# LittleWat/multichannel-semseg-with-uda

Hardware: AMD Instinct MI355X
Metric: RGB-D img/s (6x480x640) MCD train step, drn_d_38 (higher is better)
Workload: dtype f32 (operands split 2-way into scaled fp16, 3 cross terms on the fp16 MFMA pipe, fp32 accumulate)

## Files before the change

multichannel-semseg-with-uda_amd/csrc/conv_gemm_split_pp.hip:

```cpp
#include <cstdlib>
#include <type_traits>

#include "conv_split_params.h"
#include "options.h"

namespace {

template <class P, bool DGRAD, int WM, int WN, int QM, int QN>
__global__ __launch_bounds__(512, (WM * WN <= 4 ? 4 : 2)) void conv_gemm_split_pp_kernel(ConvSplitParams p) {
  static_assert(QM * QN == 4, "four waves per group");
  constexpr int WAVES_N = QN;
  constexpr int BM = 2 * QM * WM * 32, BN = QN * WN * 32, NT = 512, NS = 3;
  constexpr int NP = P::NP;
  constexpr int NPU = P::NPU;
  constexpr int NQ = 2 * NP;
  typedef typename P::frag frag;
  constexpr int A_UNITS = 2 * NPU * BM;
  constexpr int A_DMAS = (A_UNITS + NT - 1) / NT;
  constexpr int B_UNITS = 2 * NPU * BN;
  constexpr int B_DMAS = (B_UNITS + NT - 1) / NT;
  constexpr int KDEEP = P::KDEEP;
  static_assert(KDEEP == 1 || NPU == 1, "deep K-steps use the slots of the pieces the policy does not stage");
  constexpr int A_SUB = 2 * NPU * BM > A_DMAS * NT ? 2 * NPU * BM : A_DMAS * NT;
  constexpr int B_SUB = 2 * NPU * BN > B_DMAS * NT ? 2 * NPU * BN : B_DMAS * NT;
  constexpr int DMA_PER_STEP = KDEEP * (A_DMAS + B_DMAS);
  constexpr int A_BYTES = KDEEP > 1 ? KDEEP * A_SUB * 16 : (NQ * BM > A_DMAS * NT ? NQ * BM : A_DMAS * NT) * 16;
  constexpr int B_BYTES = KDEEP > 1 ? KDEEP * B_SUB * 16 : (NQ * BN > B_DMAS * NT ? NQ * BN : B_DMAS * NT) * 16;
  constexpr bool SAMEPX = (NT % BN) == 0;
  constexpr int NPX = SAMEPX ? 1 : B_DMAS;
  constexpr bool LANEHALF = (BN % 64) != 0;
  static_assert(BM % 64 == 0 && (2 * BN) % 64 == 0 && (!LANEHALF || !SAMEPX),
                "every wave issues the same number of DMAs (the waits are counted); a wave's units share a piece");
  static_assert(NS * (A_BYTES + B_BYTES) <= 160 * 1024, "LDS");

  __shared__ __attribute__((aligned(16))) unsigned char smem[NS * (A_BYTES + B_BYTES)];
  unsigned char* As = smem;
  unsigned char* Bs = smem + NS * A_BYTES;

  const int t = threadIdx.x;
  const int lane = t & 63;
  const int wave = __builtin_amdgcn_readfirstlane(t >> 6);
  const int grp_id = wave >> 2;
  const int wm = grp_id * QM + (wave & 3) / QN;
  const int wn = (wave & 3) % QN;
  const int l31 = lane & 31, lh = lane >> 5;

  const int m_tiles = p.Mp / BM;
  const int n_tiles = p.tile_n1;
  const int per_xcd = (n_tiles - p.tile_n0 + 7) >> 3;
  const int xcd = blockIdx.x & 7;
  const int slot = blockIdx.x >> 3;
  const int tile_m = slot % m_tiles;
  const int tile_n = p.tile_n0 + xcd * per_xcd + slot / m_tiles;
  if (tile_n >= n_tiles) return;

  const int HWd = p.Hd * p.Wd;
  const int HWs = p.Hs * p.Ws;
  constexpr unsigned OOB = 0x80000000u;
  __amdgpu_buffer_rsrc_t cb_rs[NPU];
#pragma unroll
  for (int pc = 0; pc < NPU; ++pc)
    cb_rs[pc] = __builtin_amdgcn_make_buffer_rsrc((void*)((const char*)p.src_cb + pc * p.cb_piece_stride), 0, p.cb_bytes, 0x00020000);
  const __amdgpu_buffer_rsrc_t wp_rs = __builtin_amdgcn_make_buffer_rsrc((void*)p.wp, 0, p.wp_bytes, 0x00020000);
  const int C8 = p.Cs >> 3;
  const int taps = p.KH * p.KW;
  unsigned valid_mask[NPX], vbase[NPX];
  int khalf[NPX];
#pragma unroll
  for (int x = 0; x < NPX; ++x) {
    const int plane_l = (t + x * NT) / BN;
    khalf[x] = LANEHALF ? (plane_l & 1) : 0;
    const int bj = (t + x * NT) % BN;
    const int pix = tile_n * BN + bj;
    const bool pv = pix < p.P;
    int pn = 0, py = 0, px = 0;
    if (pv) {
      pn = pix / HWd;
      const int rem = pix - pn * HWd;
      py = rem / p.Wd;
      px = rem - py * p.Wd;
    }
    const unsigned pix_base = (unsigned)pn * (unsigned)C8 * (unsigned)HWs;
    unsigned vm = 0;
    for (int q = 0; q < taps; ++q) {
      const int ky = q / p.KW, kx = q - ky * p.KW;
      const int sy = DGRAD ? py + p.pad - ky * p.dil : py * p.stride + ky * p.dil - p.pad;
      const int sx = DGRAD ? px + p.pad - kx * p.dil : px * p.stride + kx * p.dil - p.pad;
      vm |= (pv && sy >= 0 && sy < p.Hs && sx >= 0 && sx < p.Ws ? 1u : 0u) << q;
    }
    valid_mask[x] = (LANEHALF && plane_l >= 2 * NPU) ? 0u : vm;
    vbase[x] = DGRAD ? pix_base + (unsigned)(py * p.Ws + px) : pix_base + (unsigned)(py * p.stride * p.Ws + px * p.stride);
    if (LANEHALF) vbase[x] += (unsigned)(khalf[x] * HWs);
  }

  unsigned a_voff[A_DMAS];
#pragma unroll
  for (int i = 0; i < A_DMAS; ++i) {
    const int id = t + i * NT;
    const int plane = id / BM;
    const int m = id - plane * BM;
    a_voff[i] = id < A_UNITS ? ((unsigned)plane * (unsigned)p.Mp + (unsigned)m) * 16u : OOB;
  }

  int l_tap = 0, l_c0 = 0, l_ky = 0, l_kx = 0, l_kstep = 0;
  auto issue_sub = [&](int buf, int d) {
#if defined(__HIP_DEVICE_COMPILE__)
    const int a_soff = (l_kstep * NQ * p.Mp + tile_m * BM) * 16;
    unsigned char* adst = As + buf * A_BYTES + (d * A_SUB + wave * 64) * 16;
#pragma unroll
    for (int i = 0; i < A_DMAS; ++i)
      __builtin_amdgcn_raw_ptr_buffer_load_lds(wp_rs, (__attribute__((address_space(3))) void*)(adst + i * NT * 16), 16, a_voff[i], a_soff, 0, 0);
    const int rel = DGRAD ? (p.pad - l_ky * p.dil) * p.Ws + (p.pad - l_kx * p.dil) : (l_ky * p.dil - p.pad) * p.Ws + (l_kx * p.dil - p.pad);
    unsigned voff[NPX];
#pragma unroll
    for (int x = 0; x < NPX; ++x) {
      bool ok = ((valid_mask[x] >> l_tap) & 1u) != 0;
      if (LANEHALF) ok = ok && (l_c0 >> 3) + khalf[x] < C8;
      voff[x] = ok ? (vbase[x] + (unsigned)rel) * 16u : OOB;
    }
#if defined(MCD_ABLATE) && (MCD_ABLATE & 64)
    if (l_tap == 0)
#endif
#pragma unroll
    for (int i = 0; i < B_DMAS; ++i) {
      const int unit0 = wave * 64 + i * NT;
      const int plane = LANEHALF ? 2 * (unit0 / (2 * BN)) : unit0 / BN;
      const int grp = (l_c0 >> 3) + (plane & 1);
      const int soff = (grp < C8 && plane < 2 * NPU) ? grp * HWs * 16 : 0x7FFFFFFF;
      unsigned char* bdst = Bs + buf * B_BYTES + (d * B_SUB + unit0) * 16;
      const __amdgpu_buffer_rsrc_t rs = (NPU > 1 && plane >= 2) ? cb_rs[NPU - 1] : cb_rs[0];
      __builtin_amdgcn_raw_ptr_buffer_load_lds(rs, (__attribute__((address_space(3))) void*)bdst, 16, voff[SAMEPX ? 0 : i], soff, 0, 0);
    }
#else
    (void)buf;
    (void)d;
#endif
  };
  auto advance = [&]() {
    ++l_kstep;
    ++l_tap;
    if (++l_kx == p.KW) {
      l_kx = 0;
      ++l_ky;
    }
    if (l_tap == taps) {
      l_tap = 0;
      l_kx = 0;
      l_ky = 0;
      l_c0 += 16;
    }
  };

  auto issue = [&](int buf) {
    issue_sub(buf, 0);
    if constexpr (KDEEP > 1) {
#pragma unroll
      for (int d = 1; d < KDEEP; ++d) {
        advance();
        issue_sub(buf, d);
      }
    }
  };

  f32x16 acc[WM][WN];
#pragma unroll
  for (int i = 0; i < WM; ++i)
#pragma unroll
    for (int j = 0; j < WN; ++j)
#pragma unroll
      for (int r = 0; r < 16; ++r) acc[i][j][r] = 0.f;

  const int nsteps = taps * (p.Kp / 16) / KDEEP;
  issue(0);
  if (nsteps > 1) {
    advance();
    issue(1);
  }
  asm volatile("s_waitcnt vmcnt(0) lgkmcnt(0)\n\ts_barrier" ::: "memory");
  if (grp_id == 1) __builtin_amdgcn_s_barrier();

  frag fa[KDEEP > 1 ? KDEEP : NP][WM], fb[KDEEP > 1 ? KDEEP : NP][WN];
  int cur = 0, nxt2 = 2;
  for (int s = 0; s < nsteps; ++s) {
    const unsigned char* a_base = As + cur * A_BYTES + (lh * BM + wm * (32 * WM) + l31) * 16;
    const unsigned char* b_base = Bs + cur * B_BYTES + (lh * BN + wn * (32 * WN) + l31) * 16;
    if constexpr (KDEEP > 1) {
#pragma unroll
      for (int d = 0; d < KDEEP; ++d) {
#pragma unroll
        for (int i = 0; i < WM; ++i) fa[d][i] = *reinterpret_cast<const frag*>(a_base + (d * A_SUB + i * 32) * 16);
#pragma unroll
        for (int j = 0; j < WN; ++j) fb[d][j] = *reinterpret_cast<const frag*>(b_base + (d * B_SUB + j * 32) * 16);
      }
    } else {
#pragma unroll
    for (int pc = 0; pc < NPU; ++pc) {
#pragma unroll
      for (int i = 0; i < WM; ++i) fa[pc][i] = *reinterpret_cast<const frag*>(a_base + (pc * 2 * BM + i * 32) * 16);
#pragma unroll
      for (int j = 0; j < WN; ++j) fb[pc][j] = *reinterpret_cast<const frag*>(b_base + (pc * 2 * BN + j * 32) * 16);
    }
    }
    __builtin_amdgcn_sched_barrier(0);
    if (s + 2 < nsteps) {
      advance();
      issue(nxt2);
      asm volatile("s_waitcnt vmcnt(%0) lgkmcnt(0)\n\ts_barrier" ::"n"(DMA_PER_STEP) : "memory");
    } else {
      asm volatile("s_waitcnt vmcnt(0) lgkmcnt(0)\n\ts_barrier" ::: "memory");
    }
    __builtin_amdgcn_sched_barrier(0);
    if constexpr (KDEEP > 1) {
#pragma unroll
      for (int d = 0; d < KDEEP; ++d)
#pragma unroll
        for (int i = 0; i < WM; ++i)
#pragma unroll
          for (int j = 0; j < WN; ++j) acc[i][j] = P::mfma(fa[d][i], fb[d][j], acc[i][j]);
    } else {
#pragma unroll
    for (int tm = 0; tm < P::NTERMS; ++tm)
#pragma unroll
      for (int i = 0; i < WM; ++i)
#pragma unroll
        for (int j = 0; j < WN; ++j) acc[i][j] = P::mfma(fa[P::TA[tm]][i], fb[P::TB[tm]][j], acc[i][j]);
    }
    __builtin_amdgcn_sched_barrier(0);
    asm volatile("s_barrier" ::: "memory");
    cur = cur == 2 ? 0 : cur + 1;
    nxt2 = nxt2 == 2 ? 0 : nxt2 + 1;
  }
  if (grp_id == 0) __builtin_amdgcn_s_barrier();

  if constexpr (P::SCALED) {
    const float osc = mcd_scale_of_bound(*p.src_bound) * mcd_scale_of_bound(*p.w_bound);
#pragma unroll
    for (int i = 0; i < WM; ++i)
#pragma unroll
      for (int j = 0; j < WN; ++j)
#pragma unroll
        for (int r = 0; r < 16; ++r) acc[i][j][r] *= osc;
  }
  const int m_wave = tile_m * BM + wm * (32 * WM);
  const int p_wave = tile_n * BN + wn * (32 * WN);
  if (!DGRAD && p.bias != nullptr) {
#pragma unroll
    for (int i = 0; i < WM; ++i)
#pragma unroll
      for (int r = 0; r < 16; ++r) {
        const int m = m_wave + i * 32 + (r & 3) + 8 * (r >> 2) + 4 * lh;
        const float bv = (m < p.M) ? p.bias[m] : 0.f;
#pragma unroll
        for (int j = 0; j < WN; ++j) acc[i][j][r] += bv;
      }
  }
// ... 223 lines not shown
  return math == MCDSEG_MATH_F16X1 && !small && mcd_opt(MCD_OPT_PP_DEEP) != 0 && ((q.KH * q.KW * (q.Kp / 16)) & 1) == 0;
}

template <int WM, int WN, int QM, int QN>
void launch_math(const ConvSplitParams& q, int math, bool dgrad, hipStream_t st) {
  if constexpr (!(WM == 2 && WN == 2 && QM == 2 && QN == 2)) {
    if (deep_applies<WM, WN, QM, QN>(q, math)) {
      if (dgrad)
        launch_tile<SplitF16x1D, true, WM, WN, QM, QN>(q, st);
      else
        launch_tile<SplitF16x1D, false, WM, WN, QM, QN>(q, st);
      return;
    }
  }
  if (math == MCDSEG_MATH_F16X1) {
    if (dgrad)
      launch_tile<SplitF16x1, true, WM, WN, QM, QN>(q, st);
    else
      launch_tile<SplitF16x1, false, WM, WN, QM, QN>(q, st);
  } else {
    if (dgrad)
      launch_tile<SplitF16x3, true, WM, WN, QM, QN>(q, st);
    else
      launch_tile<SplitF16x3, false, WM, WN, QM, QN>(q, st);
  }
}

int pp_wide(const ConvSplitParams& p, int math, bool dgrad) {
  const int mode = pp_mode();
  if ((mode != 3 && mode != 4) || !pp_applies(p, math, dgrad, 128)) return 0;
  const int kind = (p.Mp % 256) == 0 ? 1 : 2;
  if (mode == 4) return kind;
  const int64_t fill = mcd_opt(MCD_OPT_PP_WIDE_FILL);
  if (fill > 100) return 0;
  const int64_t cus = compute_units();
  if (kind == 2) {
    if (mcd_opt(MCD_OPT_PP_WIDE128) == 0) return 0;
    const int64_t tiles = ceil_div64(p.P, 320) * (p.Mp / 128), rounds_w = ceil_div64(tiles, cus);
    return tiles * 100 >= fill * rounds_w * cus ? 2 : 0;
  }
  const int64_t m_tiles = p.Mp / 256;
  const int64_t tiles = ceil_div64(p.P, 320) * m_tiles, rounds_w = ceil_div64(tiles, cus);
  const int min_rounds = pp_min_rounds() > 1 ? pp_min_rounds() : 1;
  const int64_t rounds = (p.P / 256) * m_tiles / cus;
  if (rounds < min_rounds) {
    if (tiles * 100 >= fill * rounds_w * cus) return 1;
    const int64_t tiles_h = ceil_div64(p.P, 160) * m_tiles, rounds_h = ceil_div64(tiles_h, cus);
    return tiles_h * 100 >= fill * rounds_h * cus ? 3 : 0;
  }
  int64_t n_pp = rounds * cus / m_tiles;
  if (n_pp > p.P / 256) n_pp = p.P / 256;
  const int64_t rest = ceil_div64(p.P - n_pp * 256, 128) * m_tiles;
  return 5 * rounds_w <= 4 * rounds + 2 * ceil_div64(rest, cus) ? 1 : 0;
}

}

int mcdseg_internal_conv_pp_wide(const ConvSplitParams& p, int math, bool dgrad) { return pp_wide(p, math, dgrad); }

int mcdseg_internal_conv_pp_deep(const ConvSplitParams& p, int math) { return deep_applies<4, 2, 1, 4>(p, math) ? 1 : 0; }

int64_t mcdseg_internal_conv_pp_pixels(const ConvSplitParams& p, int math, bool dgrad) {
  const int mode = pp_mode();
  if (pp_wide(p, math, dgrad)) return p.P;
  if ((mode != 1 && mode != 3) || !pp_applies(p, math, dgrad)) return 0;
  const int64_t m_tiles = p.Mp / 256, n_full = p.P / 256, cus = compute_units();
  const int64_t rounds = n_full * m_tiles / cus;
  if (rounds < 1 || rounds < pp_min_rounds()) return 0;
  int64_t n_pp = rounds * cus / m_tiles;
  if (n_pp > n_full) n_pp = n_full;
  return n_pp * 256;
}

int mcdseg_internal_conv_pp_rest(const ConvSplitParams& p, int math, bool dgrad) {
  const int mode = pp_mode();
  if (!pp_applies(p, math, dgrad)) return 0;
  if (mode == 2) return 1;
  return mode == 3 && (p.P / 256) * (p.Mp / 256) / compute_units() >= (pp_min_rounds() > 1 ? pp_min_rounds() : 1) ? 1 : 0;
}

int mcdseg_internal_conv_pp_launch(const ConvSplitParams& p, int math, bool dgrad, int64_t pixels, hipStream_t st) {
  ConvSplitParams q = p;
  q.sub = 0;
  q.tile_n0 = 0;
  if (const int kind = pp_wide(p, math, dgrad)) {
    q.tile_n1 = ceil_div(p.P, kind == 3 ? 160 : 320);
    if (kind == 1)
      launch_math<2, 5, 2, 2>(q, math, dgrad, st);
    else if (kind == 2)
      launch_math<1, 5, 2, 2>(q, math, dgrad, st);
    else
      launch_math<1, 5, 4, 1>(q, math, dgrad, st);
    MCD_LAUNCH_CHECK("conv_gemm_split_pp (256 / 128 x 320, 256 x 160)");
    return 0;
  }
  q.tile_n1 = (int)(pixels / 256);
  launch_math<4, 2, 1, 4>(q, math, dgrad, st);
  MCD_LAUNCH_CHECK("conv_gemm_split_pp");
  return 0;
}

int mcdseg_internal_conv_pp_rest_launch(const ConvSplitParams& p, int math, bool dgrad, int64_t pix0, hipStream_t st) {
  ConvSplitParams q = p;
  q.sub = 0;
  q.tile_n0 = (int)(pix0 / 128);
  q.tile_n1 = ceil_div(p.P, 128);
  launch_math<2, 2, 2, 2>(q, math, dgrad, st);
  MCD_LAUNCH_CHECK("conv_gemm_split_pp (256 x 128)");
  return 0;
}
```

multichannel-semseg-with-uda_amd/csrc/conv_split_params.h:

```cpp
#pragma once
#include "split.h"

struct ConvSplitParams {
  const float* src;
  const void* src_cb;
  const void* wp;
  const float* src_bound;
  const float* w_bound;
  const float* bias;
  float* dst;
  float* stats;
  const float* ep_scale;
  const float* ep_shift;
  const float* ep_res;
  int ep_relu;
  int N;
  int Cs, Hs, Ws;
  int M, Hd, Wd;
  int Mp, Kp;
  int KH, KW, stride, pad, dil;
  int P;
  int src_bytes, wp_bytes, cb_bytes;
  long long cb_piece_stride;
  int sub;
  int cls_tile0[5];
  int tile_n0, tile_n1;
  int ep_res_lds;
  unsigned ep_res_bytes;
  void* dst16;
  float* dst_bound;
  const void* ep_res16;
};

typedef _Float16 mcd_f16x4 __attribute__((ext_vector_type(4)));
typedef __bf16 mcd_bf16x4 __attribute__((ext_vector_type(4)));
```

multichannel-semseg-with-uda_amd/csrc/conv_wgrad_split_pp.hip:

```cpp
#include <cstdlib>
#include <type_traits>

#include "split.h"

namespace {

struct WgradPpParams {
  const void* x_cb;
  const void* dy_cb;
  float* slab;
  int N, Cin, H, W, Cout, Ho, Wo;
  int KH, KW, stride, pad, dil;
  int co_tiles, ci_tiles;
  int tiles_x, tiles_y;
  int kt;
  int L, nwg;
  int slabs;
  int items;
  int x_cb_bytes, dy_cb_bytes;
  long long x_piece_stride, dy_piece_stride;
};

template <class P>
__global__ __launch_bounds__(512) void conv_wgrad_split_pp_kernel(WgradPpParams p) {
  static_assert(P::NP == 2, "two-piece policies");
  constexpr int WM = 4, WN = 2;
  constexpr int NP = P::NP;
  constexpr int NBLK = 2;
  typedef typename P::frag frag;
  typedef short s16x4 __attribute__((ext_vector_type(4)));
  typedef short s16x8 __attribute__((ext_vector_type(8)));
  constexpr int NDMA = 4;
  constexpr int DSTR = 1024 + 64;
  constexpr int BLKB = NDMA * DSTR;
  constexpr int UNIT = NBLK * BLKB;
  constexpr int STAGE = 2 * NP * UNIT;
  constexpr int NS = 3;
  static_assert(NS * STAGE <= 160 * 1024, "LDS");
  constexpr bool DEEP = P::KDEEP == 2 && P::NPU == 1 && NP == 2;
  constexpr int PRO = DEEP ? 4 : 2;
  __shared__ __attribute__((aligned(16))) unsigned char smem[NS * STAGE];

  const int t = threadIdx.x;
  const int lane = t & 63;
  const int wave = __builtin_amdgcn_readfirstlane(t >> 6);
  const int grp_id = wave >> 2;
  const int wm = grp_id, wn = wave & 3;
  const int l31 = lane & 31, lh = lane >> 5;
  const int T_ = p.KH * p.KW;

  const int w_id = (blockIdx.x & 7) * (gridDim.x >> 3) + (blockIdx.x >> 3);
  if (w_id >= p.nwg) return;
  const int tiles_all = p.co_tiles * p.ci_tiles * T_;
  const long long total = (long long)tiles_all * p.kt;
  long long g_next = (long long)w_id * p.L;
  long long g_end = g_next + p.L;
  if (g_end > total) g_end = total;
  int item = w_id;
  if (p.slabs > 0) {
    g_next = 0;
    g_end = item < p.items ? 1 : 0;
  }

  const int opnd = wave >> 2;
  const int piece = (wave >> 1) & 1;
  const int blk = wave & 1;
  const bool isx = opnd == 1;
  const int px = lane & 15;
  const int cgl = lane >> 4;
  const int sH = isx ? p.H : p.Ho;
  const int sW = isx ? p.W : p.Wo;
  const int sS = isx ? p.stride : 1;
  const int sC8 = (isx ? p.Cin : p.Cout) >> 3;
  const int sHW = sH * sW;
  const int bias = p.pad * 16 + 16;
  const char* sptr = (const char*)(isx ? p.x_cb : p.dy_cb) + piece * (isx ? p.x_piece_stride : p.dy_piece_stride) - bias;
  const int sbytes = (isx ? p.x_cb_bytes : p.dy_cb_bytes) + bias;
  const __amdgpu_buffer_rsrc_t rs = __builtin_amdgcn_make_buffer_rsrc((void*)sptr, 0, sbytes, 0x00020000);
  constexpr unsigned OOB = 0x80000000u;
  const int lane_x = px * sS;
  unsigned char* const unit_lds = smem + (opnd * NP + piece) * UNIT + blk * BLKB;
  const bool dma_on = piece < P::NPU;
  const int ntiles = p.tiles_x * p.tiles_y;

  const int gl = lane & 15;
  const int tq = gl >> 2, tpp = gl & 3;
  const int trow = ((((lane >> 4) & 1) * 2 + (tpp >> 1)) * DSTR) + tq * 16 + 8 * (tpp & 1) + (2 * lh) * 64;
  const int a_lane = wm * BLKB + trow;
  const int b_lane = (wn >> 1) * BLKB + (wn & 1) * 512 + trow;

  auto tr_read_at = [&](unsigned base, auto off_c) -> s16x4 {
    s16x4 v;
#if defined(__HIP_DEVICE_COMPILE__)
    asm volatile("ds_read_b64_tr_b16 %0, %1 offset:%2" : "=v"(v) : "v"(base), "n"(decltype(off_c)::value) : "memory");
#else
    (void)base;
    v = s16x4{};
#endif
    return v;
  };
  auto frag_of = [&](unsigned base, auto lo_c, auto hi_c) -> frag {
    const s16x4 lo = tr_read_at(base, lo_c);
    const s16x4 hi = tr_read_at(base, hi_c);
    const s16x8 v = {lo[0], lo[1], lo[2], lo[3], hi[0], hi[1], hi[2], hi[3]};
    return __builtin_bit_cast(frag, v);
  };
#if defined(__HIP_DEVICE_COMPILE__)
  const unsigned smem_lds = (unsigned)(size_t)(__attribute__((address_space(3))) unsigned char*)smem;
#else
  const unsigned smem_lds = 0;
#endif

  while (g_next < g_end) {
    int tile, k0, k1, slab_id;
    if (p.slabs > 0) {
      const int sl = item / tiles_all;
      tile = item - sl * tiles_all;
      k0 = sl * p.L;
      k1 = k0 + p.L < p.kt ? k0 + p.L : p.kt;
      slab_id = item;
      item += p.nwg;
      if (item >= p.items) g_next = g_end;
    } else {
      tile = (int)(g_next / p.kt);
      k0 = (int)(g_next - (long long)tile * p.kt);
      k1 = (g_end - (long long)tile * p.kt < p.kt) ? (int)(g_end - (long long)tile * p.kt) : p.kt;
      slab_id = (int)(g_next / p.L) + tile;
      g_next += k1 - k0;
    }
    const int tap = tile % T_;
    const int tile_ci = (tile / T_) % p.ci_tiles;
    const int tile_co = tile / (T_ * p.ci_tiles);
    const int ky = tap / p.KW, kx = tap - ky * p.KW;
    const int shy = isx ? ky * p.dil - p.pad : 0;
    const int shx = isx ? kx * p.dil - p.pad : 0;
    const int cg0 = (isx ? tile_ci : tile_co) * 32 + blk * 16;
    unsigned vconst[NDMA];
#pragma unroll
    for (int d = 0; d < NDMA; ++d) vconst[d] = (cg0 + d + 4 * cgl) < sC8 ? (unsigned)((d + 4 * cgl) * sHW + px * sS) * 16u : OOB;

    int l_n = k0 / ntiles;
    int l_ty = (k0 - l_n * ntiles) / p.tiles_x;
    int l_tx = k0 - l_n * ntiles - l_ty * p.tiles_x;
    auto stage_off = [](int c) { return DEEP ? (c < NS ? c * STAGE : (c - NS) * STAGE + UNIT) : c * STAGE; };
    auto issue = [&](int stage) {
#if defined(__HIP_DEVICE_COMPILE__)
      if (dma_on) {
        const int sbase = (l_n * sC8 + cg0) * sHW;
        const int iy = l_ty * sS + shy;
        const int ux = l_tx * 16 * sS + shx;
        const bool colok = (unsigned)(ux + lane_x) < (unsigned)sW;
        const int soff = ((unsigned)iy < (unsigned)sH) ? (sbase + iy * sW + ux) * 16 + bias : 0x7FFFFFFF;
#pragma unroll
        for (int d = 0; d < NDMA; ++d)
          __builtin_amdgcn_raw_ptr_buffer_load_lds(rs, (__attribute__((address_space(3))) void*)(unit_lds + stage_off(stage) + d * DSTR), 16,
                                                   colok ? vconst[d] : OOB, soff, 0, 0);
      }
#else
      (void)stage;
#endif
    };
    auto advance = [&]() {
      if (++l_tx == p.tiles_x) {
        l_tx = 0;
        if (++l_ty == p.tiles_y) {
          l_ty = 0;
          ++l_n;
        }
      }
    };

    f32x16 acc[WM][WN];
#pragma unroll
    for (int i = 0; i < WM; ++i)
#pragma unroll
      for (int j = 0; j < WN; ++j)
#pragma unroll
        for (int r = 0; r < 16; ++r) acc[i][j][r] = 0.f;

    const int nsteps = k1 - k0;
    issue(0);
#pragma unroll
    for (int a = 1; a < PRO; ++a)
      if (nsteps > a) {
        advance();
        issue(a);
      }
    asm volatile("s_waitcnt vmcnt(0) lgkmcnt(0)\n\ts_barrier" ::: "memory");
    if (grp_id == 1) __builtin_amdgcn_s_barrier();

    if constexpr (DEEP) {
      const int nint = (nsteps + 1) >> 1;
      frag fa2[2][WM], fb2[2][WN];
      int dcur = 0, dnxt = 2;
      for (int t = 0; t < nint; ++t) {
        const bool has2 = 2 * t + 1 < nsteps;
        const unsigned off0 = (unsigned)stage_off(2 * dcur), off1 = (unsigned)stage_off(2 * dcur + 1);
        const unsigned a0 = smem_lds + off0 + (unsigned)a_lane, b0 = smem_lds + off0 + (unsigned)b_lane;
        const unsigned a1 = smem_lds + off1 + (unsigned)a_lane, b1 = smem_lds + off1 + (unsigned)b_lane;
#define MCD_A2(U, BASE, I) fa2[U][I] = frag_of(BASE, std::integral_constant<int, (I) * 256>{}, std::integral_constant<int, (I) * 256 + 64>{});
#define MCD_B2(U, BASE, J) \
        fb2[U][J] = frag_of(BASE, std::integral_constant<int, NP * UNIT + (J) * 256>{}, std::integral_constant<int, NP * UNIT + (J) * 256 + 64>{});
        MCD_A2(0, a0, 0) MCD_A2(0, a0, 1) MCD_A2(0, a0, 2) MCD_A2(0, a0, 3) MCD_B2(0, b0, 0) MCD_B2(0, b0, 1)
        MCD_A2(1, a1, 0) MCD_A2(1, a1, 1) MCD_A2(1, a1, 2) MCD_A2(1, a1, 3) MCD_B2(1, b1, 0) MCD_B2(1, b1, 1)
#undef MCD_A2
#undef MCD_B2
        __builtin_amdgcn_sched_barrier(0);
        const int nx = 2 * (t + 2);
        if (nx + 1 < nsteps) {
          advance();
          issue(2 * dnxt);
          advance();
          issue(2 * dnxt + 1);
          if (dma_on)
            asm volatile("s_waitcnt vmcnt(%0) lgkmcnt(0)\n\ts_barrier" ::"n"(2 * NDMA) : "memory");
          else
            asm volatile("s_waitcnt lgkmcnt(0)\n\ts_barrier" ::: "memory");
        } else {
          if (nx < nsteps) {
            advance();
            issue(2 * dnxt);
          }
          asm volatile("s_waitcnt vmcnt(0) lgkmcnt(0)\n\ts_barrier" ::: "memory");
        }
#pragma unroll
        for (int u = 0; u < 2; ++u) {
#pragma unroll
          for (int i = 0; i < WM; ++i) asm volatile("" : "+v"(fa2[u][i]));
#pragma unroll
          for (int j = 0; j < WN; ++j) asm volatile("" : "+v"(fb2[u][j]));
        }
        __builtin_amdgcn_sched_barrier(0);
#pragma unroll
        for (int i = 0; i < WM; ++i)
#pragma unroll
          for (int j = 0; j < WN; ++j) acc[i][j] = P::mfma(fa2[0][i], fb2[0][j], acc[i][j]);
        if (has2) {
#pragma unroll
          for (int i = 0; i < WM; ++i)
#pragma unroll
            for (int j = 0; j < WN; ++j) acc[i][j] = P::mfma(fa2[1][i], fb2[1][j], acc[i][j]);
        }
        __builtin_amdgcn_sched_barrier(0);
        asm volatile("s_barrier" ::: "memory");
        dcur = dcur == 2 ? 0 : dcur + 1;
        dnxt = dnxt == 2 ? 0 : dnxt + 1;
      }
    } else {
      frag fa[NP][WM], fb[NP][WN];
      int cur = 0, nxt2 = 2;
      for (int s = 0; s < nsteps; ++s) {
        const unsigned base_a = smem_lds + (unsigned)(stage_off(cur) + a_lane), base_b = smem_lds + (unsigned)(stage_off(cur) + b_lane);
#define MCD_A_FRAG(PC, I) \
        if constexpr ((PC) < P::NPU) \
          fa[PC][I] = frag_of(base_a, std::integral_constant<int, (PC) * UNIT + (I) * 256>{}, std::integral_constant<int, (PC) * UNIT + (I) * 256 + 64>{});
#define MCD_B_FRAG(PC, J) \
        if constexpr ((PC) < P::NPU) \
          fb[PC][J] = frag_of(base_b, std::integral_constant<int, (NP + (PC)) * UNIT + (J) * 256>{}, std::integral_constant<int, (NP + (PC)) * UNIT + (J) * 256 + 64>{});
        MCD_A_FRAG(0, 0) MCD_A_FRAG(0, 1) MCD_A_FRAG(0, 2) MCD_A_FRAG(0, 3) MCD_B_FRAG(0, 0) MCD_B_FRAG(0, 1)
        MCD_A_FRAG(1, 0) MCD_A_FRAG(1, 1) MCD_A_FRAG(1, 2) MCD_A_FRAG(1, 3) MCD_B_FRAG(1, 0) MCD_B_FRAG(1, 1)
#undef MCD_A_FRAG
#undef MCD_B_FRAG
        __builtin_amdgcn_sched_barrier(0);
        if (s + 2 < nsteps) {
// ... 102 lines not shown
  constexpr int NS = 3;
  static_assert(NS * STAGE <= 160 * 1024, "LDS");
  __shared__ __attribute__((aligned(16))) unsigned char smem[NS * STAGE];

  const int t = threadIdx.x;
  const int lane = t & 63;
  const int wave = __builtin_amdgcn_readfirstlane(t >> 6);
  const int grp_id = wave >> 2;
  const int wm = grp_id, wn = wave & 3;
  const int l31 = lane & 31, lh = lane >> 5;

  const int w_id = (blockIdx.x & 7) * (gridDim.x >> 3) + (blockIdx.x >> 3);
  if (w_id >= p.nwg) return;
  const int tiles_all = p.co_tiles * p.ci_tiles * p.KH;

  const bool isx = wave >= 2;
  const int piece = isx ? ((wave - 2) & 1) : wave;
  const int kxs = isx ? ((wave - 2) >> 1) : 0;
  const int px = lane & 15;
  const int cgl = lane >> 4;
  const int sH = isx ? p.H : p.Ho;
  const int sW = isx ? p.W : p.Wo;
  const int sS = isx ? p.stride : 1;
  const int sC8 = (isx ? p.Cin : p.Cout) >> 3;
  const int sHW = sH * sW;
  const int bias = p.pad * 16 + 16;
  const char* sptr = (const char*)(isx ? p.x_cb : p.dy_cb) + piece * (isx ? p.x_piece_stride : p.dy_piece_stride) - bias;
  const int sbytes = (isx ? p.x_cb_bytes : p.dy_cb_bytes) + bias;
  const __amdgpu_buffer_rsrc_t rs = __builtin_amdgcn_make_buffer_rsrc((void*)sptr, 0, sbytes, 0x00020000);
  constexpr unsigned OOB = 0x80000000u;
  const int lane_x = px * sS;
  unsigned char* const unit_lds = smem + (isx ? (2 + piece * 3 + kxs) : piece) * BLKB;
  const bool dma_on = piece < P::NPU;
  const int ntiles = p.tiles_x * p.tiles_y;

  const int gl = lane & 15;
  const int tq = gl >> 2, tpp = gl & 3;
  const int trow = ((((lane >> 4) & 1) * 2 + (tpp >> 1)) * DSTR) + tq * 16 + 8 * (tpp & 1) + (2 * lh) * 64;
  const int a_lane = (wm * 2) * 256 + trow;
  int b_lane[WN];
#pragma unroll
  for (int j = 0; j < WN; ++j) {
    const int col0 = wn * 96 + j * 32;
    b_lane[j] = (2 + (col0 >> 7)) * BLKB + ((col0 & 127) >> 5) * 256 + trow;
  }

  auto tr_read_at = [&](unsigned base, auto off_c) -> s16x4 {
    s16x4 v;
#if defined(__HIP_DEVICE_COMPILE__)
    asm volatile("ds_read_b64_tr_b16 %0, %1 offset:%2" : "=v"(v) : "v"(base), "n"(decltype(off_c)::value) : "memory");
#else
    (void)base;
    v = s16x4{};
#endif
    return v;
  };
  auto frag_of = [&](unsigned base, auto lo_c, auto hi_c) -> frag {
    const s16x4 lo = tr_read_at(base, lo_c);
    const s16x4 hi = tr_read_at(base, hi_c);
    const s16x8 v = {lo[0], lo[1], lo[2], lo[3], hi[0], hi[1], hi[2], hi[3]};
    return __builtin_bit_cast(frag, v);
  };
#if defined(__HIP_DEVICE_COMPILE__)
  const unsigned smem_lds = (unsigned)(size_t)(__attribute__((address_space(3))) unsigned char*)smem;
#else
  const unsigned smem_lds = 0;
#endif

  for (int item = w_id; item < p.items; item += p.nwg) {
    const int sl = item / tiles_all;
    const int tile = item - sl * tiles_all;
    const int k0 = sl * p.L;
    const int k1 = k0 + p.L < p.kt ? k0 + p.L : p.kt;
    const int ky = tile % p.KH;
    const int tile_ci = (tile / p.KH) % p.ci_tiles;
    const int tile_co = tile / (p.KH * p.ci_tiles);
    const int shy = isx ? ky * p.dil - p.pad : 0;
    const int shx = isx ? kxs * p.dil - p.pad : 0;
    const int cg0 = (isx ? tile_ci : tile_co) * 16;
    unsigned vconst[NDMA];
#pragma unroll
    for (int d = 0; d < NDMA; ++d) vconst[d] = (cg0 + d + 4 * cgl) < sC8 ? (unsigned)((d + 4 * cgl) * sHW + px * sS) * 16u : OOB;

    int l_n = k0 / ntiles;
    int l_ty = (k0 - l_n * ntiles) / p.tiles_x;
    int l_tx = k0 - l_n * ntiles - l_ty * p.tiles_x;
    auto issue = [&](int stage) {
#if defined(__HIP_DEVICE_COMPILE__)
      if (dma_on) {
        const int sbase = (l_n * sC8 + cg0) * sHW;
        const int iy = l_ty * sS + shy;
        const int ux = l_tx * 16 * sS + shx;
        const bool colok = (unsigned)(ux + lane_x) < (unsigned)sW;
        const int soff = ((unsigned)iy < (unsigned)sH) ? (sbase + iy * sW + ux) * 16 + bias : 0x7FFFFFFF;
#pragma unroll
        for (int d = 0; d < NDMA; ++d)
          __builtin_amdgcn_raw_ptr_buffer_load_lds(rs, (__attribute__((address_space(3))) void*)(unit_lds + stage * STAGE + d * DSTR), 16,
                                                   colok ? vconst[d] : OOB, soff, 0, 0);
      }
#else
      (void)stage;
#endif
    };
    auto advance = [&]() {
      if (++l_tx == p.tiles_x) {
        l_tx = 0;
        if (++l_ty == p.tiles_y) {
          l_ty = 0;
          ++l_n;
        }
      }
    };

    f32x16 acc[WM][WN];
#pragma unroll
    for (int i = 0; i < WM; ++i)
#pragma unroll
      for (int j = 0; j < WN; ++j)
#pragma unroll
        for (int r = 0; r < 16; ++r) acc[i][j][r] = 0.f;

    const int nsteps = k1 - k0;
    issue(0);
    if (nsteps > 1) {
      advance();
      issue(1);
    }
    asm volatile("s_waitcnt vmcnt(0) lgkmcnt(0)\n\ts_barrier" ::: "memory");
    if (grp_id == 1) __builtin_amdgcn_s_barrier();

    frag fa[NP][WM], fb[NP][WN];
    int cur = 0, nxt2 = 2;
    for (int s = 0; s < nsteps; ++s) {
      const unsigned base_a = smem_lds + (unsigned)(cur * STAGE + a_lane);
      const unsigned base_b0 = smem_lds + (unsigned)(cur * STAGE + b_lane[0]), base_b1 = smem_lds + (unsigned)(cur * STAGE + b_lane[1]),
                     base_b2 = smem_lds + (unsigned)(cur * STAGE + b_lane[2]);
#define MCD_A3_FRAG(PC, I) \
      if constexpr ((PC) < P::NPU) \
        fa[PC][I] = frag_of(base_a, std::integral_constant<int, (PC) * BLKB + (I) * 256>{}, std::integral_constant<int, (PC) * BLKB + (I) * 256 + 64>{});
#define MCD_B3_FRAG(PC, J, BASE) \
      if constexpr ((PC) < P::NPU) \
        fb[PC][J] = frag_of(BASE, std::integral_constant<int, (PC) * 3 * BLKB>{}, std::integral_constant<int, (PC) * 3 * BLKB + 64>{});
      MCD_A3_FRAG(0, 0) MCD_A3_FRAG(0, 1) MCD_B3_FRAG(0, 0, base_b0) MCD_B3_FRAG(0, 1, base_b1) MCD_B3_FRAG(0, 2, base_b2)
      MCD_A3_FRAG(1, 0) MCD_A3_FRAG(1, 1) MCD_B3_FRAG(1, 0, base_b0) MCD_B3_FRAG(1, 1, base_b1) MCD_B3_FRAG(1, 2, base_b2)
#undef MCD_A3_FRAG
#undef MCD_B3_FRAG
      __builtin_amdgcn_sched_barrier(0);
      if (s + 2 < nsteps) {
        advance();
        issue(nxt2);
        if (dma_on)
          asm volatile("s_waitcnt vmcnt(%0) lgkmcnt(0)\n\ts_barrier" ::"n"(NDMA) : "memory");
        else
          asm volatile("s_waitcnt lgkmcnt(0)\n\ts_barrier" ::: "memory");
      } else {
        asm volatile("s_waitcnt vmcnt(0) lgkmcnt(0)\n\ts_barrier" ::: "memory");
      }
#pragma unroll
      for (int pc = 0; pc < P::NPU; ++pc) {
#pragma unroll
        for (int i = 0; i < WM; ++i) asm volatile("" : "+v"(fa[pc][i]));
#pragma unroll
        for (int j = 0; j < WN; ++j) asm volatile("" : "+v"(fb[pc][j]));
      }
      __builtin_amdgcn_sched_barrier(0);
#pragma unroll
      for (int tm = 0; tm < P::NTERMS; ++tm)
#pragma unroll
        for (int i = 0; i < WM; ++i)
#pragma unroll
          for (int j = 0; j < WN; ++j) acc[i][j] = P::mfma(fa[P::TA[tm]][i], fb[P::TB[tm]][j], acc[i][j]);
      __builtin_amdgcn_sched_barrier(0);
      asm volatile("s_barrier" ::: "memory");
      cur = cur == 2 ? 0 : cur + 1;
      nxt2 = nxt2 == 2 ? 0 : nxt2 + 1;
    }
    if (grp_id == 0) __builtin_amdgcn_s_barrier();

    float* out = p.slab + (size_t)item * (128 * 384);
#pragma unroll
    for (int i = 0; i < WM; ++i)
#pragma unroll
      for (int r = 0; r < 16; ++r) {
        const int row = wm * 64 + i * 32 + (r & 3) + 8 * (r >> 2) + 4 * lh;
#pragma unroll
        for (int j = 0; j < WN; ++j) out[row * 384 + wn * 96 + j * 32 + l31] = acc[i][j][r];
      }
  }
}

__global__ __launch_bounds__(256) void wgrad_reduce_rt_kernel(const float* __restrict__ slab, float* __restrict__ dw, int Cout, int Cin, int KH,
                                                             int ci_tiles, int slabs, int tiles_all, const float* __restrict__ x_bound,
                                                             const float* __restrict__ dy_bound) {
  __shared__ float stage[64 * 33];
  const int T = KH * 3;
  const int co = blockIdx.y;
  const int ci0 = blockIdx.x * 64;
  const int lane = threadIdx.x & 63, wave = threadIdx.x >> 6;
  const int ci = ci0 + lane;
  const double sc = x_bound != nullptr ? (double)mcd_scale_of_bound(*x_bound) * (double)mcd_scale_of_bound(*dy_bound) : 1.0;
  const int nci = Cin - ci0 < 64 ? Cin - ci0 : 64;
  const size_t SL = (size_t)tiles_all * (128 * 384);
  for (int tap = wave; tap < T; tap += 4) {
    const int ky = tap / 3, kx = tap - ky * 3;
    const int tile = ((co >> 7) * ci_tiles + (ci0 >> 7)) * KH + ky;
    double s = 0.0;
// ... 10 lines not shown
      for (; k < slabs; ++k, src += SL) s += (double)*src;
    }
    stage[lane * T + tap] = (float)(s * sc);
  }
  __syncthreads();
  float* out = dw + ((size_t)co * Cin + ci0) * T;
  for (int i = threadIdx.x; i < nci * T; i += 256) out[i] = stage[i];
}

int pp_compute_units() {
  if (mcd_opt(MCD_OPT_WGRAD_PP_CUS) > 0) return (int)mcd_opt(MCD_OPT_WGRAD_PP_CUS);
  if (mcd_opt(MCD_OPT_PP_CUS) > 0) return (int)mcd_opt(MCD_OPT_PP_CUS);
  static const int n = [] {
    int dev = 0, cus = 0;
    if (hipGetDevice(&dev) != hipSuccess || hipDeviceGetAttribute(&cus, hipDeviceAttributeMultiprocessorCount, dev) != hipSuccess || cus <= 0)
      cus = 256;
    return cus;
  }();
  return n;
}

}

int mcdseg_internal_wgrad_pp_plan(const mcdseg_conv_desc* d, int math, int* L, size_t* slab_floats, int* slabs_out) {
  if (mcd_opt(MCD_OPT_WGRAD_PP) == 0) return 0;
  const bool stream_k = mcd_opt(MCD_OPT_WGRAD_PP) == 1;
  if (slabs_out) *slabs_out = 0;
  if (mcd_storage_math(math) != MCDSEG_MATH_F16X3 || (d->Cin & 7) || (d->Cout & 7) || d->Cin < 129 || d->Cout < 129) return 0;
  const int T = d->KH * d->KW;
  if (T > 32 || d->pad > 128) return 0;
  const int64_t co_tiles = ceil_div(d->Cout, 256), ci_tiles = ceil_div(d->Cin, 256);
  if (co_tiles * 256 - d->Cout >= 128 || ci_tiles * 256 - d->Cin >= 128) return 0;
  const int64_t kt = (int64_t)d->N * ceil_div(d->Wo, 16) * d->Ho;
  const int64_t tiles = co_tiles * ci_tiles * T, total = tiles * kt;
  int64_t nwg = pp_compute_units();
  if (total < nwg * 32) return 0;
  if (!stream_k) {
    int64_t best_r = 0, best_ls = 0, best_ns = 0;
    double best_eff = 0.0;
    for (int64_t r = 1; r <= 4; ++r) {
      int64_t ns = r * nwg / tiles;
      if (ns < 1) continue;
      if (ns > kt / 32) ns = kt / 32;
      if (ns < 1) continue;
      const int64_t ls = ceil_div64(kt, ns);
      ns = ceil_div64(kt, ls);
      const double eff = (double)total / ((double)nwg * (double)(ceil_div64(ns * tiles, nwg) * ls));
      if (eff > best_eff + 0.02 || best_r == 0) best_r = r, best_ls = ls, best_ns = ns, best_eff = eff;
      if (best_eff >= 0.95) break;
    }
    if (best_r > 0 && best_eff >= 0.80) {
      const int64_t items = best_ns * tiles;
      const int64_t rounds = ceil_div64(items, nwg);
      if (L) *L = (int)best_ls;
      if (slabs_out) *slabs_out = (int)best_ns;
      if (slab_floats) *slab_floats = (size_t)items * 256 * 256;
      return (int)ceil_div64(items, rounds);
    }
  }
  const int64_t l = ceil_div64(total, nwg);
  if (l > kt) return 0;
  nwg = ceil_div64(total, l);
  if (L) *L = (int)l;
  if (slab_floats) *slab_floats = (size_t)(nwg + tiles + 1) * 256 * 256;
  return (int)nwg;
}

int mcdseg_internal_wgrad_pp_launch(const mcdseg_conv_desc* d, int math, const void* x_cb, const float* x_bound, const void* dy_cb,
                                    const float* dy_bound, float* dw, float* slab, hipStream_t st) {
  WgradPpParams p;
  int L = 0, slabs = 0;
  const int nwg = mcdseg_internal_wgrad_pp_plan(d, math, &L, nullptr, &slabs);
  MCD_REQUIRE(nwg > 0, "conv_wgrad_split_pp: the geometry has no stream-K plan");
  const int64_t xb = (int64_t)d->N * d->Cin * d->H * d->W * 2, yb = (int64_t)d->N * d->Cout * d->Ho * d->Wo * 2;
  MCD_REQUIRE(xb + 4096 < (1ll << 31) && yb + 4096 < (1ll << 31) && (d->Ncb == 0 || d->Ncb >= d->N),
              "conv_wgrad_split_pp: pre-split operands need < 2 GiB per operand piece and Ncb >= N");
  p.x_cb = x_cb; p.dy_cb = dy_cb; p.slab = slab;
  p.N = d->N; p.Cin = d->Cin; p.H = d->H; p.W = d->W; p.Cout = d->Cout; p.Ho = d->Ho; p.Wo = d->Wo;
  p.KH = d->KH; p.KW = d->KW; p.stride = d->stride; p.pad = d->pad; p.dil = d->dil;
  p.co_tiles = ceil_div(d->Cout, 256); p.ci_tiles = ceil_div(d->Cin, 256);
  p.tiles_x = ceil_div(d->Wo, 16); p.tiles_y = d->Ho;
  p.kt = d->N * p.tiles_x * p.tiles_y;
  p.L = L; p.nwg = nwg;
  p.slabs = slabs; p.items = slabs * p.co_tiles * p.ci_tiles * d->KH * d->KW;
  p.x_cb_bytes = (int)xb; p.dy_cb_bytes = (int)yb;
  p.x_piece_stride = math == MCDSEG_MATH_F16X1 ? 0 : (long long)(d->Ncb ? d->Ncb : d->N) * d->Cin * d->H * d->W * 2;
  p.dy_piece_stride = math == MCDSEG_MATH_F16X1 ? 0 : (long long)(d->Ncb ? d->Ncb : d->N) * d->Cout * d->Ho * d->Wo * 2;
  const dim3 grid((unsigned)(8 * ceil_div(nwg, 8)));
  if (math == MCDSEG_MATH_F16X1 && mcd_opt(MCD_OPT_WGRAD_PP_DEEP) != 0)
    hipLaunchKernelGGL(conv_wgrad_split_pp_kernel<SplitF16x1D>, grid, dim3(512), 0, st, p);
  else if (math == MCDSEG_MATH_F16X1)
    hipLaunchKernelGGL(conv_wgrad_split_pp_kernel<SplitF16x1>, grid, dim3(512), 0, st, p);
  else
    hipLaunchKernelGGL(conv_wgrad_split_pp_kernel<SplitF16x3>, grid, dim3(512), 0, st, p);
  MCD_LAUNCH_CHECK("conv_wgrad_split_pp");
  const int T = d->KH * d->KW;
  MCD_REQUIRE(T <= 33, "conv_wgrad_split_pp: more than 33 taps");
  hipLaunchKernelGGL(wgrad_reduce_sk_kernel, dim3((unsigned)ceil_div(d->Cin, 64), (unsigned)d->Cout), dim3(256), 0, st, (const float*)slab, dw, d->Cout,
                     d->Cin, T, p.ci_tiles, p.kt, L, slabs, p.co_tiles * p.ci_tiles * T, x_bound, dy_bound);
  MCD_LAUNCH_CHECK("wgrad_reduce_sk");
  return 0;
}

int mcdseg_internal_wgrad_pp3_plan(const mcdseg_conv_desc* d, int math, int* L, size_t* slab_floats, int* slabs_out) {
  if (mcd_opt(MCD_OPT_WGRAD_PP3) == 0) return 0;
  if (slabs_out) *slabs_out = 0;
  if (mcd_storage_math(math) != MCDSEG_MATH_F16X3 || (d->Cin & 7) || (d->Cout & 7)) return 0;
  const int lo = d->Cin < d->Cout ? d->Cin : d->Cout;
  if (lo <= 64 || (d->Cin >= 129 && d->Cout >= 129)) return 0;
  if (d->KW != 3 || d->KH > 10 || d->pad > 128) return 0;
  const int64_t co_tiles = ceil_div(d->Cout, 128), ci_tiles = ceil_div(d->Cin, 128);
  if (4 * (int64_t)d->Cout * d->Cin < 3 * (co_tiles * 128) * (ci_tiles * 128)) return 0;
  const int64_t kt = (int64_t)d->N * ceil_div(d->Wo, 16) * d->Ho;
  const int64_t tiles = co_tiles * ci_tiles * d->KH, total = tiles * kt;
  const int64_t nwg = pp_compute_units();
  if (total < nwg * 32) return 0;
  int64_t best_r = 0, best_ls = 0, best_ns = 0;
  double best_eff = 0.0;
  for (int64_t r = 1; r <= 4; ++r) {
    int64_t ns = r * nwg / tiles;
    if (ns < 1) continue;
    if (ns > kt / 32) ns = kt / 32;
    if (ns < 1) continue;
    const int64_t ls = ceil_div64(kt, ns);
    ns = ceil_div64(kt, ls);
    const double eff = (double)total / ((double)nwg * (double)(ceil_div64(ns * tiles, nwg) * ls));
    if (eff > best_eff + 0.02 || best_r == 0) best_r = r, best_ls = ls, best_ns = ns, best_eff = eff;
    if (best_eff >= 0.95) break;
  }
  if (best_r == 0 || best_eff < 0.80) return 0;
  const int64_t items = best_ns * tiles;
  const int64_t rounds = ceil_div64(items, nwg);
  if (items * 128 * 384 >= (1ll << 31)) return 0;
  if (L) *L = (int)best_ls;
  if (slabs_out) *slabs_out = (int)best_ns;
  if (slab_floats) *slab_floats = (size_t)items * 128 * 384;
  return (int)ceil_div64(items, rounds);
}

int mcdseg_internal_wgrad_pp3_launch(const mcdseg_conv_desc* d, int math, const void* x_cb, const float* x_bound, const void* dy_cb,
                                     const float* dy_bound, float* dw, float* slab, hipStream_t st) {
  WgradPpParams p;
  int L = 0, slabs = 0;
  const int nwg = mcdseg_internal_wgrad_pp3_plan(d, math, &L, nullptr, &slabs);
  MCD_REQUIRE(nwg > 0 && slabs > 0, "conv_wgrad_split_pp3: the geometry has no plan");
  const int64_t xb = (int64_t)d->N * d->Cin * d->H * d->W * 2, yb = (int64_t)d->N * d->Cout * d->Ho * d->Wo * 2;
  MCD_REQUIRE(xb + 4096 < (1ll << 31) && yb + 4096 < (1ll << 31) && (d->Ncb == 0 || d->Ncb >= d->N),
              "conv_wgrad_split_pp3: pre-split operands need < 2 GiB per operand piece and Ncb >= N");
  p.x_cb = x_cb; p.dy_cb = dy_cb; p.slab = slab;
  p.N = d->N; p.Cin = d->Cin; p.H = d->H; p.W = d->W; p.Cout = d->Cout; p.Ho = d->Ho; p.Wo = d->Wo;
  p.KH = d->KH; p.KW = d->KW; p.stride = d->stride; p.pad = d->pad; p.dil = d->dil;
  p.co_tiles = ceil_div(d->Cout, 128); p.ci_tiles = ceil_div(d->Cin, 128);
  p.tiles_x = ceil_div(d->Wo, 16); p.tiles_y = d->Ho;
  p.kt = d->N * p.tiles_x * p.tiles_y;
  p.L = L; p.nwg = nwg;
  p.slabs = slabs; p.items = slabs * p.co_tiles * p.ci_tiles * d->KH;
  p.x_cb_bytes = (int)xb; p.dy_cb_bytes = (int)yb;
  p.x_piece_stride = math == MCDSEG_MATH_F16X1 ? 0 : (long long)(d->Ncb ? d->Ncb : d->N) * d->Cin * d->H * d->W * 2;
  p.dy_piece_stride = math == MCDSEG_MATH_F16X1 ? 0 : (long long)(d->Ncb ? d->Ncb : d->N) * d->Cout * d->Ho * d->Wo * 2;
  const dim3 grid((unsigned)(8 * ceil_div(nwg, 8)));
  if (math == MCDSEG_MATH_F16X1)
    hipLaunchKernelGGL(conv_wgrad_split_pp3_kernel<SplitF16x1>, grid, dim3(512), 0, st, p);
  else
    hipLaunchKernelGGL(conv_wgrad_split_pp3_kernel<SplitF16x3>, grid, dim3(512), 0, st, p);
  MCD_LAUNCH_CHECK("conv_wgrad_split_pp3");
  hipLaunchKernelGGL(wgrad_reduce_rt_kernel, dim3((unsigned)ceil_div(d->Cin, 64), (unsigned)d->Cout), dim3(256), 0, st, (const float*)slab, dw, d->Cout,
                     d->Cin, d->KH, p.ci_tiles, slabs, p.co_tiles * p.ci_tiles * d->KH, x_bound, dy_bound);
  MCD_LAUNCH_CHECK("wgrad_reduce_rt");
  return 0;
}
```

multichannel-semseg-with-uda_amd/csrc/options.h:

```cpp
#pragma once
#include <stdint.h>

#define MCD_OPTIONS(X)                                                                                                       \
  X(BN_STATS_ONE, 1024)                     \
  X(BN_REVERSE, 1)                              \
  X(BN_V4, 1)                                         \
  X(BIGTILE_MIN_SLOTS, 1024)                               \
  X(WIDETILE_MIN_SLOTS, 1024)                                                                 \
  X(DGRAD_INTERLEAVE, 1)       \
  X(DGRAD_ADD_LDS, 1)                   \
  X(PACK_BLOCKS, 192)                               \
  X(PP_MIN_ROUNDS, 2)          \
  X(PP_CUS, 0)                 \
  X(PINGPONG, 3)               \
  X(PP_WIDE_FILL, 80)                               \
  X(PP_WIDE128, 1)                                                                                \
  X(PP_DEEP, 1)                \
  X(THIN_WINDOW, 1)                                                           \
  X(WGRAD_WGS, 1024)                                  \
  X(WGRAD_THIN_TR, 1)                                                               \
  X(WGRAD_TR64, 1)                                                    \
  X(WGRAD_BIG, 1)                                                                       \
  X(WGRAD_PP_CUS, 0)                          \
  X(WGRAD_PP, 2)                                          \
  X(WGRAD_PP3, 1)                                                                 \
  X(WGRAD_PP_DEEP, 1)          \
  X(UP8_LOSS_DMA, 1)                                  \
  X(UP8_BAND_ROWS, -1)

enum McdOpt {
#define X(name, def) MCD_OPT_##name,
  MCD_OPTIONS(X)
#undef X
      MCD_OPT_COUNT
};

int64_t mcd_opt(McdOpt which);
```

Before: 81.69.

## Skip dead kernel taps and out-of-bounds rows in conv GEMM and wgrad

```diff
diff --git a/multichannel-semseg-with-uda_amd/csrc/conv_gemm_split_pp.hip b/multichannel-semseg-with-uda_amd/csrc/conv_gemm_split_pp.hip
--- a/multichannel-semseg-with-uda_amd/csrc/conv_gemm_split_pp.hip
+++ b/multichannel-semseg-with-uda_amd/csrc/conv_gemm_split_pp.hip
@@ -102,6 +102,25 @@
     a_voff[i] = id < A_UNITS ? ((unsigned)plane * (unsigned)p.Mp + (unsigned)m) * 16u : OOB;
   }
 
+  const unsigned all_taps = taps >= 32 ? 0xFFFFFFFFu : (1u << taps) - 1u;
+  unsigned live = all_taps;
+  if (p.skip_dead) {
+    unsigned m = 0;
+#pragma unroll
+    for (int x = 0; x < NPX; ++x) m |= valid_mask[x];
+#pragma unroll
+    for (int o = 32; o > 0; o >>= 1) m |= __shfl_xor(m, o, 64);
+    volatile unsigned* live_w = reinterpret_cast<volatile unsigned*>(As + 2 * A_BYTES);
+    if (lane == 0) live_w[wave] = m;
+    __syncthreads();
+    m = 0;
+#pragma unroll
+    for (int w = 0; w < NT / 64; ++w) m |= live_w[w];
+    m = __builtin_amdgcn_readfirstlane(m);
+    const int live_steps = __builtin_popcount(m) * (p.Kp / 16);
+    if (m != 0 && (KDEEP == 1 || (live_steps % KDEEP) == 0)) live = m;
+  }
+
   int l_tap = 0, l_c0 = 0, l_ky = 0, l_kx = 0, l_kstep = 0;
   auto issue_sub = [&](int buf, int d) {
 #if defined(__HIP_DEVICE_COMPILE__)
@@ -136,7 +155,7 @@
     (void)d;
 #endif
   };
-  auto advance = [&]() {
+  auto next_step = [&]() {
     ++l_kstep;
     ++l_tap;
     if (++l_kx == p.KW) {
@@ -150,6 +169,11 @@
       l_c0 += 16;
     }
   };
+  auto advance = [&]() {
+    do next_step();
+    while (((live >> l_tap) & 1u) == 0);
+  };
+  while (((live >> l_tap) & 1u) == 0) next_step();
 
   auto issue = [&](int buf) {
     issue_sub(buf, 0);
@@ -170,7 +194,7 @@
 #pragma unroll
       for (int r = 0; r < 16; ++r) acc[i][j][r] = 0.f;
 
-  const int nsteps = taps * (p.Kp / 16) / KDEEP;
+  const int nsteps = __builtin_popcount(live) * (p.Kp / 16) / KDEEP;
   issue(0);
   if (nsteps > 1) {
     advance();
@@ -560,6 +584,7 @@
 int mcdseg_internal_conv_pp_launch(const ConvSplitParams& p, int math, bool dgrad, int64_t pixels, hipStream_t st) {
   ConvSplitParams q = p;
   q.sub = 0;
+  q.skip_dead = mcd_opt(MCD_OPT_SKIP_DEAD_TAPS) != 0 ? 1 : 0;
   q.tile_n0 = 0;
   if (const int kind = pp_wide(p, math, dgrad)) {
     q.tile_n1 = ceil_div(p.P, kind == 3 ? 160 : 320);
@@ -581,6 +606,7 @@
 int mcdseg_internal_conv_pp_rest_launch(const ConvSplitParams& p, int math, bool dgrad, int64_t pix0, hipStream_t st) {
   ConvSplitParams q = p;
   q.sub = 0;
+  q.skip_dead = mcd_opt(MCD_OPT_SKIP_DEAD_TAPS) != 0 ? 1 : 0;
   q.tile_n0 = (int)(pix0 / 128);
   q.tile_n1 = ceil_div(p.P, 128);
   launch_math<2, 2, 2, 2>(q, math, dgrad, st);
diff --git a/multichannel-semseg-with-uda_amd/csrc/conv_split_params.h b/multichannel-semseg-with-uda_amd/csrc/conv_split_params.h
--- a/multichannel-semseg-with-uda_amd/csrc/conv_split_params.h
+++ b/multichannel-semseg-with-uda_amd/csrc/conv_split_params.h
@@ -30,6 +30,7 @@
   void* dst16;
   float* dst_bound;
   const void* ep_res16;
+  int skip_dead;
 };
 
 typedef _Float16 mcd_f16x4 __attribute__((ext_vector_type(4)));
diff --git a/multichannel-semseg-with-uda_amd/csrc/conv_wgrad_split_pp.hip b/multichannel-semseg-with-uda_amd/csrc/conv_wgrad_split_pp.hip
--- a/multichannel-semseg-with-uda_amd/csrc/conv_wgrad_split_pp.hip
+++ b/multichannel-semseg-with-uda_amd/csrc/conv_wgrad_split_pp.hip
@@ -19,6 +19,40 @@
   int items;
   int x_cb_bytes, dy_cb_bytes;
   long long x_piece_stride, dy_piece_stride;
+  int skip_dead;
+};
+
+struct LiveRows {
+  int lo, hi, tiles_x, ntiles;
+  __device__ LiveRows(const WgradPpParams& p, int ky) : lo(0), hi(p.tiles_y), tiles_x(p.tiles_x), ntiles(p.tiles_x * p.tiles_y) {
+    if (!p.skip_dead) return;
+    const int sh = ky * p.dil - p.pad;
+    if (sh < 0) lo = (-sh + p.stride - 1) / p.stride;
+    const int last = p.H - 1 - sh;
+    const int h = last < 0 ? 0 : last / p.stride + 1;
+    if (h < hi) hi = h;
+    if (lo > hi) lo = hi;
+  }
+  __device__ int before(int k) const {
+    const int n = k / ntiles;
+    const int ty = (k - n * ntiles) / tiles_x;
+    const int tx = k - n * ntiles - ty * tiles_x;
+    const int done = ty < lo ? 0 : (ty < hi ? ty - lo : hi - lo);
+    return (n * (hi - lo) + done) * tiles_x + (ty >= lo && ty < hi ? tx : 0);
+  }
+  __device__ void first(int k, int& n, int& ty, int& tx) const {
+    n = k / ntiles;
+    ty = (k - n * ntiles) / tiles_x;
+    tx = k - n * ntiles - ty * tiles_x;
+    if (ty < lo) {
+      ty = lo;
+      tx = 0;
+    } else if (ty >= hi) {
+      ty = lo;
+      tx = 0;
+      ++n;
+    }
+  }
 };
 
 template <class P>
@@ -139,9 +173,9 @@
 #pragma unroll
     for (int d = 0; d < NDMA; ++d) vconst[d] = (cg0 + d + 4 * cgl) < sC8 ? (unsigned)((d + 4 * cgl) * sHW + px * sS) * 16u : OOB;
 
-    int l_n = k0 / ntiles;
-    int l_ty = (k0 - l_n * ntiles) / p.tiles_x;
-    int l_tx = k0 - l_n * ntiles - l_ty * p.tiles_x;
+    const LiveRows rows(p, ky);
+    int l_n, l_ty, l_tx;
+    rows.first(k0, l_n, l_ty, l_tx);
     auto stage_off = [](int c) { return DEEP ? (c < NS ? c * STAGE : (c - NS) * STAGE + UNIT) : c * STAGE; };
     auto issue = [&](int stage) {
 #if defined(__HIP_DEVICE_COMPILE__)
@@ -163,8 +197,8 @@
     auto advance = [&]() {
       if (++l_tx == p.tiles_x) {
         l_tx = 0;
-        if (++l_ty == p.tiles_y) {
-          l_ty = 0;
+        if (++l_ty == rows.hi) {
+          l_ty = rows.lo;
           ++l_n;
         }
       }
@@ -178,8 +212,8 @@
 #pragma unroll
         for (int r = 0; r < 16; ++r) acc[i][j][r] = 0.f;
 
-    const int nsteps = k1 - k0;
-    issue(0);
+    const int nsteps = rows.before(k1) - rows.before(k0);
+    if (nsteps > 0) issue(0);
 #pragma unroll
     for (int a = 1; a < PRO; ++a)
       if (nsteps > a) {
@@ -448,9 +482,9 @@
 #pragma unroll
     for (int d = 0; d < NDMA; ++d) vconst[d] = (cg0 + d + 4 * cgl) < sC8 ? (unsigned)((d + 4 * cgl) * sHW + px * sS) * 16u : OOB;
 
-    int l_n = k0 / ntiles;
-    int l_ty = (k0 - l_n * ntiles) / p.tiles_x;
-    int l_tx = k0 - l_n * ntiles - l_ty * p.tiles_x;
+    const LiveRows rows(p, ky);
+    int l_n, l_ty, l_tx;
+    rows.first(k0, l_n, l_ty, l_tx);
     auto issue = [&](int stage) {
 #if defined(__HIP_DEVICE_COMPILE__)
       if (dma_on) {
@@ -471,8 +505,8 @@
     auto advance = [&]() {
       if (++l_tx == p.tiles_x) {
         l_tx = 0;
-        if (++l_ty == p.tiles_y) {
-          l_ty = 0;
+        if (++l_ty == rows.hi) {
+          l_ty = rows.lo;
           ++l_n;
         }
       }
@@ -486,8 +520,8 @@
 #pragma unroll
         for (int r = 0; r < 16; ++r) acc[i][j][r] = 0.f;
 
-    const int nsteps = k1 - k0;
-    issue(0);
+    const int nsteps = rows.before(k1) - rows.before(k0);
+    if (nsteps > 0) issue(0);
     if (nsteps > 1) {
       advance();
       issue(1);
@@ -664,6 +698,7 @@
   p.tiles_x = ceil_div(d->Wo, 16); p.tiles_y = d->Ho;
   p.kt = d->N * p.tiles_x * p.tiles_y;
   p.L = L; p.nwg = nwg;
+  p.skip_dead = mcd_opt(MCD_OPT_SKIP_DEAD_TAPS) != 0 ? 1 : 0;
   p.slabs = slabs; p.items = slabs * p.co_tiles * p.ci_tiles * d->KH * d->KW;
   p.x_cb_bytes = (int)xb; p.dy_cb_bytes = (int)yb;
   p.x_piece_stride = math == MCDSEG_MATH_F16X1 ? 0 : (long long)(d->Ncb ? d->Ncb : d->N) * d->Cin * d->H * d->W * 2;
@@ -736,6 +771,7 @@
   p.tiles_x = ceil_div(d->Wo, 16); p.tiles_y = d->Ho;
   p.kt = d->N * p.tiles_x * p.tiles_y;
   p.L = L; p.nwg = nwg;
+  p.skip_dead = mcd_opt(MCD_OPT_SKIP_DEAD_TAPS) != 0 ? 1 : 0;
   p.slabs = slabs; p.items = slabs * p.co_tiles * p.ci_tiles * d->KH;
   p.x_cb_bytes = (int)xb; p.dy_cb_bytes = (int)yb;
   p.x_piece_stride = math == MCDSEG_MATH_F16X1 ? 0 : (long long)(d->Ncb ? d->Ncb : d->N) * d->Cin * d->H * d->W * 2;
diff --git a/multichannel-semseg-with-uda_amd/csrc/options.h b/multichannel-semseg-with-uda_amd/csrc/options.h
--- a/multichannel-semseg-with-uda_amd/csrc/options.h
+++ b/multichannel-semseg-with-uda_amd/csrc/options.h
@@ -16,6 +16,7 @@
   X(PP_WIDE_FILL, 80)                               \
   X(PP_WIDE128, 1)                                                                                \
   X(PP_DEEP, 1)                \
+  X(SKIP_DEAD_TAPS, 1)         \
   X(THIN_WINDOW, 1)                                                           \
   X(WGRAD_WGS, 1024)                                  \
   X(WGRAD_THIN_TR, 1)                                                               \
```

Result: faster. 82.91, median of 6 (+1.5%).
